# y-scope/pinot

Measured on AMD Instinct MI355X. Metric: scanned rows/sec + achieved HBM GB/s, filtered SUM on 1B-row segment, higher is better.
Workload: dtype int64

## Files before the change

### pinot_amd/csrc/pg_engine.hip

```cpp
#include <hip/hip_runtime.h>

#include <algorithm>
#include <chrono>
#include <array>
#include <atomic>
#include <condition_variable>
#include <functional>
#include <memory>
#include <cmath>
#include <cstdarg>
#include <cstdio>
#include <cstdlib>
#include <cstring>
#include <limits>
#include <mutex>
#include <string>
#include <thread>
#include <vector>

#include "../../include/pinot_gpu.h"
#include "pg_device.h"
#include "pg_filter_stats.h"
#include "pg_filter_fsm.h"
#include "pg_fsm_kernels.h"
#include "pg_kernels.h"
#include "pg_launch.h"
#include "pg_rank_image.h"
#include "pg_raw_set_table.h"

namespace {

using namespace pg;

thread_local std::string g_error;

pg_status fail(pg_status st, const char* fmt, ...) {
  char buf[1024];
  va_list ap;
  va_start(ap, fmt);
  vsnprintf(buf, sizeof(buf), fmt, ap);
  va_end(ap);
  g_error = buf;
  return st;
}

#define HIP_TRY(expr)                                                                                  \
  do {                                                                                                 \
    hipError_t _e = (expr);                                                                            \
    if (_e != hipSuccess)                                                                              \
      return fail(_e == hipErrorOutOfMemory ? PG_ERR_OUT_OF_MEMORY : PG_ERR_DEVICE, "%s failed: %s (%s:%d)", #expr, \
                  hipGetErrorString(_e), __FILE__, __LINE__);                                          \
  } while (0)

struct Engine {
  bool initialized = false;
  std::atomic<uint64_t> epoch{0};
  int device = 0;
  int blocks_per_cu = 0;
  bool raw64_coalesced = true;
  int wide_plane = -1;
  bool partition_stats_cache = true;
  bool partition_packed = true;
  bool plane_async = true;
  bool staged_h2d = true;
  long long exact_stats_docs = 64ll << 20;
  int flags = 0;
  bool use_dma = true;
  int value_plane = -1;
  int tile_steps = 0;
  bool double_buffer = false;
  bool direct_result = true;
  int fold_finalize = -1;
  int fold_one_counter = 1;
  bool poll_result = true;
  bool distinct_lds = true;
  bool set_lds = true;
  bool lane_skip = true;
  bool batch_blocks_per_cu_forced = false;
  int batch_blocks_per_cu = 4;
  bool scan_raw = true;
  bool scan_raw_set = true;
  int scan_simple_valid = 1;
  bool scan_simple = true;
  bool scan_sparse = true;
  bool lean_batch = true;
  bool partition_two_level = true;
  bool fsm_perm = true;
  int index_and_waves = 0;
  bool batch_index = true;
  bool index_gather = true;
  bool fsm_fused = true;
  bool fsm_stats = true;
  bool fsm_episodes = true;
  bool plan_cache = true;
  bool group_publish = true;
  bool batch_more = true;
  bool group_one_launch = true;
  bool batch_group = true;
  bool batch_hist = true;
  bool batch_launch = true;
  bool leap2 = true;
  int sparse_lanes = 32;
  bool plane_gcd = true;
  bool scan_private = true;
  bool group_private = true;
  int group_log_replicas = 3;
  bool group_pack = true;
  bool scan_typed_private = true;
  bool scan_narrow_single = true;
  bool scan_narrow = true;
  bool group_partition = true;
  long long partition_min_docs = 1ll << 22;
  unsigned long long group_table_bytes = 64ull << 30;
  int hist = -1;
  int hist_blocks = 0;
  bool hist_guard = false;
  int hist_bits = 0;
  int group_waves = 0;
  int physical_devices = 1;
  int logical_devices = 1;
  std::mutex mu;
};
Engine g_engine;
inline int phys_device(int logical) { return (g_engine.logical_devices > g_engine.physical_devices && g_engine.physical_devices > 0) ? logical % g_engine.physical_devices : logical; }
inline bool device_id_ok(int id) {
  if (id < 0) return false;
  if (g_engine.initialized) return id < g_engine.logical_devices;
  int n = 0;
  return hipGetDeviceCount(&n) == hipSuccess && id < n;
}

inline uint32_t be32(const uint8_t* p) { return ((uint32_t)p[0] << 24) | ((uint32_t)p[1] << 16) | ((uint32_t)p[2] << 8) | (uint32_t)p[3]; }
inline uint32_t le16(const uint8_t* p) { return (uint32_t)p[0] | ((uint32_t)p[1] << 8); }
inline uint32_t le32(const uint8_t* p) { return (uint32_t)p[0] | ((uint32_t)p[1] << 8) | ((uint32_t)p[2] << 16) | ((uint32_t)p[3] << 24); }

struct ColumnDev {
  std::string name;
  int stored_type = 0, encoding = 0, bits = 0, cardinality = 0;
  uint8_t* d_fwd_alloc = nullptr;
  uint8_t* d_fwd = nullptr;
  size_t fwd_alloc_bytes = 0;
  int32_t* d_dict = nullptr;
  std::vector<int32_t> h_dict;
  int vkind = kValI32;
  int64_t value_base = 0;
  std::vector<double> h_dict_f64;
  std::vector<int64_t> h_dict_i64;
  unsigned long long* d_dict64 = nullptr;
  uint8_t* d_inv = nullptr;
  uint64_t inv_size = 0;
  DevContainer* d_dir = nullptr;
  std::vector<DevContainer> h_dir;
  std::vector<int64_t> posting_first;
  std::vector<int64_t> posting_docs;
  unsigned long long* d_null_bitmap = nullptr;
  int nullkey_column = -1;
  int keyimage_column = -1;
  int64_t raw_min = 0, raw_max = -1;
  int key_image_of = -1;
  int64_t key_base = 0;
  int key_image_state = 0;
  bool rank_image = false;
  std::vector<unsigned long long> h_rank_keys;
  unsigned long long* d_rank_dict = nullptr;
  bool borrows_dictionary = false;
// ... 1542 lines not shown
  return v;
}

bool dict_ends_in_nan(const ColumnDev& col) {
  return col.encoding == PG_FWD_FIXED_BIT_DICT && (col.vkind == kValF64 || col.vkind == kValF32) && !col.h_dict_f64.empty() && std::isnan(col.h_dict_f64.back());
}
double group_key64_to_double(const ColumnDev& col, long long key, bool is_min) {
  if (col.vkind != kValI64 && key == (is_min ? 0x7FFFFFFFFFFFFFFFll : (long long)0x8000000000000000ull))
    return is_min ? std::numeric_limits<double>::infinity() : -std::numeric_limits<double>::infinity();
  return key64_to_double(col, key);
}

inline void cpu_relax() {
#if defined(__x86_64__) || defined(__i386__)
  __builtin_ia32_pause();
#elif defined(__aarch64__)
  asm volatile("yield" ::: "memory");
#else
  std::this_thread::yield();
#endif
}

template <typename Done>
pg_status wait_polled(hipStream_t stream, long long docs, Done&& done) {
  long long spins = 0;
  std::chrono::steady_clock::time_point until;
  while (!done()) {
    cpu_relax();
    if ((++spins & 0x3FF) != 0) continue;
    const auto now = std::chrono::steady_clock::now();
    if (spins == 0x400) { until = now + std::chrono::nanoseconds(300'000 + docs / 1000); continue; }
    if (now >= until || hipStreamQuery(stream) != hipErrorNotReady) { HIP_TRY(hipStreamSynchronize(stream)); break; }
  }
  __atomic_thread_fence(__ATOMIC_ACQUIRE);
  return PG_OK;
}

}

extern "C" {

const char* pg_last_error(void) { return g_error.c_str(); }
const char* pg_version(void) { return "pinot_amd 0.1 (gfx950)"; }

pg_status pg_init(const pg_config* config) {
  std::lock_guard<std::mutex> lk(g_engine.mu);
  if (config && config->abi_version != PG_ABI_VERSION) return fail(PG_ERR_INVALID_ARGUMENT, "ABI version mismatch: got %d, built %d", config->abi_version, PG_ABI_VERSION);
  int count = 0;
  hipError_t e = hipGetDeviceCount(&count);
  if (e != hipSuccess || count == 0) return fail(PG_ERR_DEVICE, "no HIP device available: %s", hipGetErrorString(e));
  g_engine.physical_devices = count;
  const char* ald = getenv("PINOT_GPU_ALIAS_DEVICES");
  g_engine.logical_devices = (ald && atoi(ald) > count) ? std::min(atoi(ald), 64) : count;
  int dev = config ? config->device_id : 0;
  if (dev < 0 || dev >= g_engine.logical_devices) return fail(PG_ERR_INVALID_ARGUMENT, "device %d out of range (have %d)", dev, g_engine.logical_devices);
  g_engine.device = dev;
  g_engine.blocks_per_cu = config ? config->blocks_per_cu : 0;
  g_engine.flags = config ? config->flags : 0;
  const char* nodma = getenv("PINOT_GPU_NO_DMA");
  g_engine.use_dma = !(nodma && nodma[0] == '1');
  const char* vp = getenv("PINOT_GPU_VALUE_PLANE");
  g_engine.value_plane = vp ? atoi(vp) : -1;
  const char* db = getenv("PINOT_GPU_DOUBLE_BUFFER");
  g_engine.double_buffer = db && db[0] == '1';
  const char* drv = getenv("PINOT_GPU_DIRECT_RESULT");
  g_engine.direct_result = !(drv && drv[0] == '0');
  const char* ffz = getenv("PINOT_GPU_FOLD_FINALIZE");
  g_engine.fold_finalize = ffz ? (ffz[0] == '0' ? 0 : 1) : -1;
  const char* foc = getenv("PINOT_GPU_FOLD_ONE_COUNTER");
  g_engine.fold_one_counter = foc ? (foc[0] == '0' ? 0 : 1) : 1;
  const char* prs = getenv("PINOT_GPU_POLL_RESULT");
  g_engine.poll_result = !(prs && prs[0] == '0');
  const char* lsk = getenv("PINOT_GPU_LANE_SKIP");
  g_engine.lane_skip = !(lsk && lsk[0] == '0');
  const char* bbc = getenv("PINOT_GPU_BATCH_BLOCKS_PER_CU");
  g_engine.batch_blocks_per_cu_forced = bbc != nullptr;
  g_engine.batch_blocks_per_cu = (bbc && atoi(bbc) > 0) ? atoi(bbc) : 4;
  const char* ssp = getenv("PINOT_GPU_SCAN_SPARSE");
  g_engine.scan_sparse = !(ssp && ssp[0] == '0');
  const char* ssm = getenv("PINOT_GPU_SCAN_SIMPLE");
  g_engine.scan_simple = !(ssm && ssm[0] == '0');
  const char* ssv = getenv("PINOT_GPU_SCAN_SIMPLE_VALID");
  g_engine.scan_simple_valid = ssv ? (ssv[0] == '0' ? 0 : (ssv[0] == '2' ? 2 : 1)) : 1;
  const char* srw = getenv("PINOT_GPU_SCAN_RAW");
  g_engine.scan_raw = !(srw && srw[0] == '0');
  const char* srs = getenv("PINOT_GPU_SCAN_RAW_SET");
  g_engine.scan_raw_set = !(srs && srs[0] == '0');
  const char* bla = getenv("PINOT_GPU_BATCH_LAUNCH");
  g_engine.batch_launch = !(bla && bla[0] == '0');
  auto env_on = [](const char* name) { const char* v = getenv(name); return !(v && v[0] == '0'); };
  g_engine.lean_batch = env_on("PINOT_GPU_LEAN_BATCH");
  g_engine.set_lds = env_on("PINOT_GPU_SET_LDS");
  g_engine.distinct_lds = env_on("PINOT_GPU_DISTINCT_LDS");
  g_engine.partition_two_level = env_on("PINOT_GPU_PARTITION_TWO_LEVEL");
  g_engine.fsm_perm = env_on("PINOT_GPU_FSM_PERM");
  g_engine.fsm_stats = env_on("PINOT_GPU_FSM_STATS");
  g_engine.fsm_fused = env_on("PINOT_GPU_FSM_FUSED");
  g_engine.fsm_episodes = env_on("PINOT_GPU_FSM_EPISODES");
  g_engine.index_gather = env_on("PINOT_GPU_INDEX_GATHER");
  g_engine.batch_index = env_on("PINOT_GPU_BATCH_INDEX");
  { const char* iaw = getenv("PINOT_GPU_INDEX_AND_WAVES"); g_engine.index_and_waves = iaw ? std::max(-64, std::min(32, atoi(iaw))) : 0; }
  g_engine.group_one_launch = env_on("PINOT_GPU_GROUP_ONE_LAUNCH");
  g_engine.plan_cache = env_on("PINOT_GPU_PLAN_CACHE");
  g_engine.group_publish = env_on("PINOT_GPU_GROUP_PUBLISH");
  const char* bmo = getenv("PINOT_GPU_BATCH_MORE");
  g_engine.batch_more = !(bmo && bmo[0] == '0');
  const char* bgr = getenv("PINOT_GPU_BATCH_GROUP");
  g_engine.batch_group = !(bgr && bgr[0] == '0');
  const char* bhi = getenv("PINOT_GPU_BATCH_HIST");
  g_engine.batch_hist = !(bhi && bhi[0] == '0');
  const char* lp2 = getenv("PINOT_GPU_LEAP2");
  g_engine.leap2 = !(lp2 && lp2[0] == '0');
  const char* spl = getenv("PINOT_GPU_SPARSE_LANES");
  g_engine.sparse_lanes = spl ? std::max(0, std::min(64, atoi(spl))) : 32;
  const char* pgv = getenv("PINOT_GPU_PLANE_GCD");
  g_engine.plane_gcd = !(pgv && pgv[0] == '0');
  const char* spv = getenv("PINOT_GPU_SCAN_PRIVATE");
  g_engine.scan_private = !(spv && spv[0] == '0');
  const char* gpv = getenv("PINOT_GPU_GROUP_PRIVATE");
  g_engine.group_private = !(gpv && gpv[0] == '0');
  const char* grv = getenv("PINOT_GPU_GROUP_REPLICAS");
  g_engine.group_log_replicas = grv ? std::max(0, std::min(4, atoi(grv))) : 3;
  const char* stp = getenv("PINOT_GPU_SCAN_TYPED_PRIVATE");
  g_engine.scan_typed_private = !(stp && stp[0] == '0');
  const char* gpt = getenv("PINOT_GPU_GROUP_PARTITION");
  g_engine.group_partition = !(gpt && gpt[0] == '0');
  g_engine.partition_min_docs = (gpt && gpt[0] == 'f') ? 0 : (1ll << 22);
  const char* sns = getenv("PINOT_GPU_SCAN_NARROW_SINGLE");
  g_engine.scan_narrow_single = !(sns && sns[0] == '0');
  const char* snw = getenv("PINOT_GPU_SCAN_NARROW");
  g_engine.scan_narrow = !(snw && snw[0] == '0');
  const char* gtb = getenv("PINOT_GPU_GROUP_TABLE_BYTES");
  g_engine.group_table_bytes = (gtb && atoll(gtb) > 0) ? (unsigned long long)atoll(gtb) : (64ull << 30);
  const char* gpk = getenv("PINOT_GPU_GROUP_PACK");
  g_engine.group_pack = !(gpk && gpk[0] == '0');
  const char* gw = getenv("PINOT_GPU_GROUP_WAVES");
  g_engine.group_waves = (gw && atoi(gw) > 0) ? atoi(gw) : 0;
  const char* hs = getenv("PINOT_GPU_HIST");
  g_engine.hist = hs ? atoi(hs) : -1;
  const char* hbl = getenv("PINOT_GPU_HIST_BLOCKS");
  g_engine.hist_blocks = (hbl && atoi(hbl) > 0) ? atoi(hbl) : 0;
  const char* hg = getenv("PINOT_GPU_HIST_GUARD");
  g_engine.hist_guard = hg && hg[0] == '1';
  const char* hb = getenv("PINOT_GPU_HIST_BITS");
  g_engine.hist_bits = (hb && (atoi(hb) == 8 || atoi(hb) == 16)) ? atoi(hb) : 0;
  const char* ts = getenv("PINOT_GPU_TILE_STEPS");
  g_engine.tile_steps = (ts && (atoi(ts) == 16 || atoi(ts) == 32)) ? atoi(ts) : 0;
  g_engine.raw64_coalesced = true; g_engine.wide_plane = -1; g_engine.partition_stats_cache = true; g_engine.partition_packed = true;
  g_engine.plane_async = true; g_engine.staged_h2d = true; g_engine.exact_stats_docs = 64ll << 20;
  const char* r64 = getenv("PINOT_GPU_RAW64_COALESCED");
  if (r64) g_engine.raw64_coalesced = atoi(r64) != 0;
  const char* wpl = getenv("PINOT_GPU_WIDE_PLANE");
  if (wpl) g_engine.wide_plane = atoi(wpl);
  const char* psc = getenv("PINOT_GPU_PARTITION_STATS_CACHE");
  if (psc) g_engine.partition_stats_cache = atoi(psc) != 0;
  const char* ppk = getenv("PINOT_GPU_PARTITION_PACKED");
  if (ppk) g_engine.partition_packed = atoi(ppk) != 0;
  const char* pas = getenv("PINOT_GPU_PLANE_ASYNC");
  if (pas) g_engine.plane_async = atoi(pas) != 0;
  const char* sh2d = getenv("PINOT_GPU_STAGED_H2D");
  if (sh2d) g_engine.staged_h2d = atoi(sh2d) != 0;
  {
    uint64_t budget = config ? config->plane_budget_bytes : 0;
    const char* pb = getenv("PINOT_GPU_PLANE_BUDGET_BYTES");
    if (pb) budget = strtoull(pb, nullptr, 10);
    if (budget == 0) {
// ... 681 lines not shown
  std::shared_ptr<IndexAndParams> and_params;
  uint32_t and_windows = 0;
  size_t hist_lds = 0;
  int hist_cw = 0, hist_col = -1;
  std::string key;
  uint64_t engine_epoch = 0, plane_epoch = 0;
  std::shared_ptr<const OwnedQuery> query;
};
struct Deferred {
  std::shared_ptr<const LoweredItem> item;
  std::unique_ptr<PlaneHold> planes;
  bool cacheable = false;
  bool single = false;
};

static bool query_key(const pg_query* q, std::string* key) {
  key->clear();
  if (q->num_filter_nodes < 0 || q->num_predicates < 0 || q->num_aggregations < 0 || q->num_group_by < 0) return false;
  if ((q->num_filter_nodes > 0 && !q->filter) || (q->num_predicates > 0 && !q->predicates) || (q->num_aggregations > 0 && !q->aggregations) ||
      (q->num_group_by > 0 && !q->group_by_columns)) return false;
  const int32_t head[6] = {q->num_filter_nodes, q->num_predicates, q->num_aggregations, q->num_group_by, q->num_groups_limit, q->flags};
  key->append(reinterpret_cast<const char*>(head), sizeof(head));
  key->append(reinterpret_cast<const char*>(q->filter), sizeof(pg_filter_node) * (size_t)q->num_filter_nodes);
  for (int i = 0; i < q->num_predicates; ++i) {
    const pg_predicate& pr = q->predicates[i];
    if (pr.num_set_words < 0 || (pr.num_set_words > 0 && !pr.set_words)) { key->clear(); return false; }
    const int64_t fields[8] = {pr.kind, pr.column, pr.eval, pr.exclusive, pr.lo, pr.hi, pr.num_set_words, pr.reserved};
    key->append(reinterpret_cast<const char*>(fields), sizeof(fields));
    key->append(reinterpret_cast<const char*>(pr.set_words), sizeof(uint32_t) * (size_t)pr.num_set_words);
  }
  key->append(reinterpret_cast<const char*>(q->aggregations), sizeof(pg_aggregation) * (size_t)q->num_aggregations);
  key->append(reinterpret_cast<const char*>(q->group_by_columns), sizeof(int32_t) * (size_t)q->num_group_by);
  return true;
}

static std::shared_ptr<const OwnedQuery> own_query(const pg_query* q) {
  auto o = std::make_shared<OwnedQuery>();
  o->q = *q;
  if (q->num_filter_nodes > 0) o->filter.assign(q->filter, q->filter + q->num_filter_nodes);
  if (q->num_predicates > 0) o->predicates.assign(q->predicates, q->predicates + q->num_predicates);
  o->set_words.resize(o->predicates.size());
  for (size_t i = 0; i < o->predicates.size(); ++i) {
    pg_predicate& pr = o->predicates[i];
    if (pr.num_set_words > 0) { o->set_words[i].assign(pr.set_words, pr.set_words + pr.num_set_words); pr.set_words = o->set_words[i].data(); }
    else pr.set_words = nullptr;
  }
  if (q->num_aggregations > 0) o->aggregations.assign(q->aggregations, q->aggregations + q->num_aggregations);
  o->q.filter = o->filter.empty() ? nullptr : o->filter.data();
  o->q.predicates = o->predicates.empty() ? nullptr : o->predicates.data();
  o->q.aggregations = o->aggregations.empty() ? nullptr : o->aggregations.data();
  if (q->num_group_by > 0) o->group_by.assign(q->group_by_columns, q->group_by_columns + q->num_group_by);
  o->q.group_by_columns = o->group_by.empty() ? nullptr : o->group_by.data();
  return o;
}

static pg_status prepare_fsm_side(pg_segment* seg, ExecCtx* ctx, const pg::fstats::Fsm& fsm, FsmSide* side);
static pg_status device_fsm_filter_stats(pg_segment* seg, ExecCtx* ctx, const pg_query* q, const FsmSide& side, pg_result* out);
struct ExecTrace {
  std::chrono::steady_clock::time_point t[6];
  bool seen[6];
};
static thread_local ExecTrace t_exec_trace;
static bool exec_trace_on() { static const bool on = getenv("PINOT_GPU_EXEC_TRACE") != nullptr; return on; }
static inline void exec_mark(int i) {
  if (!exec_trace_on()) return;
  t_exec_trace.t[i] = std::chrono::steady_clock::now();
  t_exec_trace.seen[i] = true;
}

static pg_status execute_impl(pg_segment* seg, const pg_query* q, pg_result* out, unsigned long long* d_out_bitmap_request,
                              uint64_t* host_bitmap, int64_t host_bitmap_words, int64_t* out_cardinality, bool allow_metadata_plan = true,
                              Deferred* defer = nullptr, FsmSide* side = nullptr);

enum class ScanKernel { Hist, Narrow, NarrowSingle, Sparse, Simple, SimpleSet, SimpleValid, Raw, RawSet, PrivateFsm, Private, PrivateTyped, Distinct, GroupDistinct, Agg };
static const struct { int id; bool writes_leaves; } kScanKernels[] = {
  {PG_KERNEL_SCAN_HIST, true}, {PG_KERNEL_SCAN_NARROW, true}, {PG_KERNEL_SCAN_NARROW, false}, {PG_KERNEL_SCAN_SPARSE, false}, {PG_KERNEL_SCAN_SIMPLE, false},
  {PG_KERNEL_SCAN_SIMPLE, false}, {PG_KERNEL_SCAN_SIMPLE_VALID, false}, {PG_KERNEL_SCAN_RAW, false}, {PG_KERNEL_SCAN_RAW_SET, false}, {PG_KERNEL_SCAN_PRIVATE, false}, {PG_KERNEL_SCAN_PRIVATE, true},
  {PG_KERNEL_SCAN_PRIVATE_TYPED, true}, {PG_KERNEL_SCAN_DISTINCT, true}, {PG_KERNEL_GROUP_DISTINCT, true}, {PG_KERNEL_SCAN_AGG, false}};
static_assert(sizeof(kScanKernels) / sizeof(kScanKernels[0]) == (size_t)ScanKernel::Agg + 1, "one row per ScanKernel");
struct ScanChoice {
  ScanKernel kernel = ScanKernel::Agg, general = ScanKernel::Agg;
  int hist_slot = -1, hist_cw = 0;
  bool hist_guarded = false;
};
static ScanChoice choose_scan_kernel(const pg_segment* seg, const Lowered& lw, int hist_col, bool typed, bool want_bitmap, bool want_result) {
  const PlanParams& pl = lw.plan; const ScanParams& sp = lw.sp;
  const bool profile = (g_engine.flags & PG_CFG_PROFILE_WAVES) != 0;
  ScanChoice k;
  auto pick = [&k](ScanKernel kernel) { k.kernel = kernel; return k; };
  if (sp.num_nodes == 1 && sp.nodes[0].op == PG_FILTER_LEAF && sp.nodes[0].kind == kLeafRawSet) { k.general = ScanKernel::Private; return pick(ScanKernel::RawSet); }
  if (!lw.distinct_slots.empty()) { k.general = ScanKernel::Private; return pick(lw.distinct_key_slots.empty() ? ScanKernel::Distinct : ScanKernel::GroupDistinct); }
  bool private_leaves = true;
  for (int l = 0; l < pl.num_leaves; ++l) private_leaves &= pl.leaves[l].kind <= kLeafBitmap || pl.leaves[l].kind == kLeafDocRange;
  bool lane_private = g_engine.scan_private && !typed && !profile && private_leaves;
  for (int i = 0; i < pl.num_agg_cols && hist_col >= 0; ++i) if (lw.col_of_slot[(size_t)pl.agg_cols[i].col] == hist_col * 2) k.hist_slot = i;
  for (int i = 0; i < pl.num_agg_cols && lane_private; ++i) {
    const DevColumn& c = pl.cols[pl.agg_cols[i].col];
    lane_private = !c.is_raw && c.vkind == kValI32 && c.bits <= 31 && (!pl.agg_cols[i].need_sum || c.is_plane || i == k.hist_slot);
  }
  const bool hist = lane_private && k.hist_slot == 0 && pl.num_agg_cols == 1;
  if (k.hist_slot >= 0 && !hist) lane_private = false;
  bool lane_typed = g_engine.scan_private && g_engine.scan_typed_private && !lane_private && pl.num_agg_cols > 0 && !profile && private_leaves;
  for (int i = 0; i < pl.num_agg_cols && lane_typed; ++i) {
    const DevColumn& c = pl.cols[pl.agg_cols[i].col];
    lane_typed = c.is_raw || (c.vkind != kValI32 && c.bits <= 31);
  }
  k.general = k.kernel = lane_private ? ScanKernel::Private : (lane_typed ? ScanKernel::PrivateTyped : ScanKernel::Agg);
  if (hist) {
    k.hist_cw = hist_counter_bits(seg->cols[(size_t)hist_col]);
    k.hist_guarded = std::max(__atomic_load_n(&seg->cols[(size_t)hist_col].hist_tier, __ATOMIC_RELAXED), g_engine.hist_guard ? 1 : 0) >= 1 && k.hist_cw < 32;
    return pick(ScanKernel::Hist);
  }
  if (k.general == ScanKernel::Agg) return k;
  if (g_engine.scan_narrow && lane_private && pl.num_agg_cols == 0 && lw.tile_list == nullptr && sp.num_nodes > 0 && !(want_result && lw.stats_leap2_flagged)) {
    bool narrow = true; int depth = 0, max_depth = 0;
    for (int n = 0; n < sp.num_nodes && narrow; ++n) {
      const DevNode& dn = sp.nodes[n];
      if (dn.op == PG_FILTER_LEAF) {
        narrow = dn.kind == kLeafMatchAll || dn.kind == kLeafMatchNone || ((dn.kind == kLeafDictRange || (dn.kind == kLeafDictSet && g_engine.set_lds)) && dn.bits >= 1 && dn.bits <= kNarrowMaxBits);
        depth++;
      } else if (dn.op != PG_FILTER_NOT) depth -= dn.num_children - 1;
      max_depth = std::max(max_depth, depth);
    }
    if (narrow && max_depth <= kNarrowStack)
      return pick(g_engine.scan_narrow_single && sp.num_nodes == 1 && sp.nodes[0].kind == kLeafDictRange ? ScanKernel::NarrowSingle : ScanKernel::Narrow);
  }
  if (g_engine.scan_sparse && lane_private && !want_bitmap && pl.num_agg_cols > 0 && lw.tile_list != nullptr && sp.num_nodes == 1 && sp.nodes[0].kind == kLeafBitmap &&
      sp.nodes[0].exclusive == 0) return pick(ScanKernel::Sparse);
  if (g_engine.scan_simple_valid != 0 && g_engine.scan_simple && lane_private && !want_bitmap && lw.tile_list == nullptr && lw.side == nullptr && lw.valid_leaf >= 0 &&
      pl.num_agg_cols <= 1 && !lw.stats_leap2_flagged && (sp.num_nodes == 1 || sp.num_nodes == 3)) {
    const DevNode& v = sp.nodes[0];
    const DevNode* range = sp.num_nodes == 3 ? &sp.nodes[1] : nullptr;
    const DevAggCol* vac = pl.num_agg_cols == 1 ? &sp.agg_cols[0] : nullptr;
    bool valid = v.op == PG_FILTER_LEAF && v.kind == kLeafBitmap && v.exclusive == 0 && v.set_words == reinterpret_cast<const uint32_t*>(pl.leaves[lw.valid_leaf].bitmap) &&
                 (range != nullptr || vac != nullptr);
    if (valid && range != nullptr)
      valid = sp.nodes[2].op == PG_FILTER_AND && sp.nodes[2].num_children == 2 && range->op == PG_FILTER_LEAF && range->kind == kLeafDictRange && range->bits >= 1 && range->bits <= kSimpleMaxBits &&
              (range->flags & kNodeLeapfrog2) == 0;
    if (valid && vac != nullptr)
      valid = vac->bits >= 1 && vac->bits <= kSimpleMaxBits && !vac->is_raw &&
              !(range != nullptr && range->fwd == vac->fwd && range->bits == vac->bits && vac->need_sum != 0 && vac->need_minmax == 0 && range->exclusive == 0);
    if (valid) return pick(ScanKernel::SimpleValid);
  }
  if (want_bitmap || lw.tile_list != nullptr || sp.num_nodes > 1 || pl.num_agg_cols > 1 || (want_result && (lw.stats_leap2_flagged || lw.stats_chain_flagged))) return k;
  const DevNode* leaf = sp.num_nodes == 1 ? &sp.nodes[0] : nullptr;
  const bool plain_leaf = leaf == nullptr || (leaf->op == PG_FILTER_LEAF && (leaf->flags & (kNodeCountEntries | kNodeLeapfrog2)) == 0);
  const DevAggCol* ac = pl.num_agg_cols == 1 ? &sp.agg_cols[0] : nullptr;
  const bool set = leaf != nullptr && leaf->op == PG_FILTER_LEAF && leaf->kind == kLeafDictSet && g_engine.set_lds && leaf->bits <= 16;
  bool simple = g_engine.scan_simple && lane_private && plain_leaf &&
                (leaf == nullptr || ((leaf->kind == kLeafDictRange || set) && leaf->bits >= 1 && leaf->bits <= kSimpleMaxBits));
  if (simple && ac != nullptr)
    simple = ac->bits >= 1 && ac->bits <= kSimpleMaxBits && !ac->is_raw && !(leaf != nullptr && leaf->fwd == ac->fwd && leaf->bits == ac->bits && ac->need_sum != 0 && ac->need_minmax == 0 && leaf->exclusive == 0);
  if (simple) return pick(set ? ScanKernel::SimpleSet : ScanKernel::Simple);
  if (g_engine.scan_raw && lw.side == nullptr && sp.num_nodes + pl.num_agg_cols >= 1 && plain_leaf && (leaf == nullptr || (leaf->kind == kLeafRawRange && leaf->fwd != nullptr)) &&
      (ac == nullptr || (ac->is_raw != 0 && ac->vkind == kValI32 && ac->is_plane == 0 && ac->bits == 32))) return pick(ScanKernel::Raw);
  return k;
}
struct ScanGrid { int blocks = 1, threads = kBlockThreads; size_t lds = 0, hist_set_off = 0; bool wide = false, distinct_lds = false; };
static void lean_grid(const pg_segment* seg, int wave_cap, ScanGrid* g) {
  const long long tiles2k = doc_tiles(seg);
  static const bool wide_ok = getenv("PINOT_GPU_WIDE_BLOCKS") && getenv("PINOT_GPU_WIDE_BLOCKS")[0] == '1';
  g->wide = wide_ok && wave_cap >= 2 * (kWideBlockThreads / 64) && tiles2k > 64 && tiles2k <= (long long)seg->num_cus * wave_cap && g_engine.blocks_per_cu <= 0;
  const int wpb = (g->wide ? kWideBlockThreads : kBlockThreads) / 64;
  int bpc = std::max(1, wave_cap / wpb);
  static const int small_bpc = getenv("PINOT_GPU_SMALL_BLOCKS_PER_CU") ? atoi(getenv("PINOT_GPU_SMALL_BLOCKS_PER_CU")) : 2;
  if (!g->wide && small_bpc > 0 && tiles2k <= 2ll * seg->num_cus * wave_cap) bpc = std::min(bpc, small_bpc);
  g->blocks = grid_blocks(seg, tiles2k, wpb, bpc);
}
static ScanGrid scan_grid(const pg_segment* seg, const ScanChoice& k, const Lowered& lw, const Geometry& geo, int num_agg_cols, int hist_col) {
  const ScanParams& sp = lw.sp;
  ScanGrid g;
  const long long tiles = doc_tiles(seg);
  const int wpb = kBlockThreads / 64, hist_waves = kHistBlockThreads / 64;
  switch (k.kernel) {
    case ScanKernel::Hist: {
      const int per_word = 32 / k.hist_cw;
      g.lds = (((size_t)(seg->cols[(size_t)hist_col].cardinality + per_word - 1) / per_word * 4) + 15) & ~(size_t)15;
      g.lds = std::max(g.lds, sizeof(BlockPartial) * (kHistBlockThreads / 64) + 16);
      if (g_engine.set_lds && g.lds + (size_t)kSetLdsWords * 4 <= 150 * 1024)
        for (int nd = 0; nd < sp.num_nodes; ++nd) if (sp.nodes[nd].op == PG_FILTER_LEAF && sp.nodes[nd].kind == kLeafDictSet) g.hist_set_off = g.lds;
      if (g.hist_set_off != 0) g.lds += (size_t)kSetLdsWords * 4;
      g.threads = kHistBlockThreads;
      g.blocks = grid_blocks(seg, tiles, hist_waves, std::max(1, std::min(waves_scan_hist(k.hist_cw, k.hist_guarded) / hist_waves, (int)((160 * 1024 - 2048) / (g.lds + 256)))));
      if (g_engine.hist_blocks > 0) g.blocks = std::min(g.blocks, g_engine.hist_blocks);
      break;
    }
    case ScanKernel::Distinct: case ScanKernel::GroupDistinct: {
      bool has_set = false;
      if (g_engine.set_lds) for (int nd = 0; nd < sp.num_nodes; ++nd) has_set |= sp.nodes[nd].op == PG_FILTER_LEAF && sp.nodes[nd].kind == kLeafDictSet;
      size_t bit_bytes = 0;
      for (int slot : lw.distinct_slots) bit_bytes += (size_t)((lw.plan.cols[slot].cardinality + 31) / 32) * 4;
      bit_bytes = (bit_bytes + 15) & ~(size_t)15;
      const size_t records = sizeof(BlockPartial) * (kHistBlockThreads / 64) + 16;
      size_t lds_tier = bit_bytes + (has_set ? (size_t)kSetLdsWords * 4 : 0);
      if (lds_tier > kLdsBudget && bit_bytes <= kLdsBudget) { has_set = false; lds_tier = bit_bytes; }
      g.distinct_lds = k.kernel == ScanKernel::Distinct && g_engine.distinct_lds && std::max(lds_tier, records) <= kLdsBudget;
      if (g.distinct_lds) {
        g.hist_set_off = has_set ? bit_bytes : 0;
        g.lds = std::max(lds_tier, records);
        g.threads = kHistBlockThreads;
        g.blocks = grid_blocks(seg, tiles, hist_waves, std::max(1, std::min(waves_scan_distinct(true) / hist_waves, (int)((160 * 1024 - 2048) / (g.lds + 256)))));
      } else {
        g.hist_set_off = has_set ? 16 : 0;
        g.lds = std::max((size_t)(has_set ? 16 + kSetLdsWords * 4 : 0), sizeof(BlockPartial) * (size_t)wpb + 16);
        g.blocks = grid_blocks(seg, tiles, wpb, std::max(1, (k.kernel == ScanKernel::Distinct ? waves_scan_distinct(false) : waves_group_distinct()) / wpb));
      }
      break;
    }
    case ScanKernel::Narrow: g.blocks = grid_blocks(seg, (tiles + kNarrowTiles - 1) / kNarrowTiles, wpb, std::max(1, waves_scan_narrow(false) / wpb)); break;
    case ScanKernel::NarrowSingle: g.blocks = grid_blocks(seg, (tiles + kNarrowSingleTiles - 1) / kNarrowSingleTiles, wpb, std::max(1, waves_scan_narrow(true) / wpb)); break;
    case ScanKernel::Sparse: g.blocks = grid_blocks(seg, tiles, wpb * kSparseTiles, std::max(1, waves_scan_sparse(num_agg_cols <= 1) / wpb)); break;
    case ScanKernel::Simple: case ScanKernel::SimpleSet: lean_grid(seg, waves_scan_simple(), &g); break;
    case ScanKernel::SimpleValid: lean_grid(seg, waves_scan_simple_valid(), &g); break;
    case ScanKernel::Raw: lean_grid(seg, waves_scan_raw(), &g); break;
    case ScanKernel::RawSet: {
      g.lds = (size_t)sp.nodes[0].set_bytes;
      int bpc = std::max(1, std::min(waves_scan_raw_set(sp.nodes[0].lo_hi) / wpb, (int)(kLdsBudget / (g.lds + 1024))));
      if (tiles <= 2ll * seg->num_cus * bpc * wpb) bpc = std::min(bpc, 2);
      g.blocks = grid_blocks(seg, tiles, wpb, bpc);
      break;
    }
    case ScanKernel::Private: g.blocks = grid_blocks(seg, tiles, wpb, std::max(1, waves_scan_private(num_agg_cols) / wpb)); break;
    case ScanKernel::PrivateTyped: g.blocks = grid_blocks(seg, tiles, wpb, std::max(1, waves_scan_private_typed(num_agg_cols) / wpb)); break;
    default: g.blocks = geo.blocks; g.threads = geo.threads; g.lds = geo.lds; break;
  }
  return g;
}
static bool scan_batch_kind(const ScanChoice& k, int num_agg_cols, BatchKind* kind) {
  const bool lean = g_engine.lean_batch;
  switch (k.kernel) {
    case ScanKernel::Hist: *kind = k.hist_cw == 8 ? BatchKind::Hist8 : (k.hist_cw == 16 ? BatchKind::Hist16 : BatchKind::Hist32); return !k.hist_guarded && g_engine.batch_hist;
    case ScanKernel::Narrow: case ScanKernel::NarrowSingle: *kind = k.kernel == ScanKernel::Narrow ? BatchKind::Narrow : BatchKind::NarrowSingle; return g_engine.batch_more;
    case ScanKernel::Simple: case ScanKernel::SimpleSet: *kind = !lean ? BatchKind::Private : (k.kernel == ScanKernel::Simple ? BatchKind::Simple : BatchKind::SimpleSet); return true;
    case ScanKernel::Raw: *kind = !lean && k.general == ScanKernel::Private ? BatchKind::Private : BatchKind::Raw; return true;
    case ScanKernel::RawSet: return false;
    case ScanKernel::SimpleValid: return false;
    case ScanKernel::PrivateFsm: case ScanKernel::Private: *kind = BatchKind::Private; return true;
    case ScanKernel::PrivateTyped: *kind = num_agg_cols <= 1 ? BatchKind::Typed1 : (num_agg_cols == 2 ? BatchKind::Typed2 : BatchKind::TypedMax); return g_engine.batch_more;
    default: return false;
  }
}
static void launch_scan_kernel(const ScanChoice& k, const ScanGrid& g, int num_agg_cols, bool typed, hipStream_t stream, const ScanParams& sp) {
  const bool one = num_agg_cols <= 1;
  const int lean_threads = g.wide ? kWideBlockThreads : kBlockThreads;
  switch (k.kernel) {
    case ScanKernel::Hist: launch_scan_hist(k.hist_cw, k.hist_guarded, g.blocks, g.lds, stream, sp); break;
    case ScanKernel::Narrow: case ScanKernel::NarrowSingle: launch_scan_narrow(k.kernel == ScanKernel::NarrowSingle, g.blocks, stream, sp); break;
    case ScanKernel::Sparse: launch_scan_sparse(one, g.blocks, stream, sp); break;
    case ScanKernel::Simple: case ScanKernel::SimpleSet: launch_scan_simple(g.blocks, lean_threads, stream, sp, k.kernel == ScanKernel::SimpleSet); break;
    case ScanKernel::SimpleValid: launch_scan_simple_valid(g.blocks, lean_threads, stream, sp, g_engine.scan_simple_valid == 2); break;
    case ScanKernel::Raw: launch_scan_raw(g.blocks, lean_threads, stream, sp); break;
    case ScanKernel::RawSet: launch_scan_raw_set(sp.nodes[0].lo_hi, g.blocks, g.lds, stream, sp); break;
    case ScanKernel::PrivateFsm: launch_scan_private_fsm(num_agg_cols, g.blocks, stream, sp); break;
    case ScanKernel::Private: launch_scan_private(num_agg_cols, g.blocks, stream, sp); break;
    case ScanKernel::PrivateTyped: launch_scan_private_typed(num_agg_cols, g.blocks, stream, sp); break;
    case ScanKernel::Agg: launch_scan_agg(g_engine.use_dma, one, typed, g.blocks, g.threads, g.lds, stream, sp); break;
    case ScanKernel::Distinct: case ScanKernel::GroupDistinct: break;
  }
}
struct QueryRun {
  pg_segment* seg; const pg_query* q; pg_result* out; ExecCtx* ctx; Deferred* defer;
  int na, ng, hist_col = -1;
  bool want_bitmap, timed, stats_is_final = false;
  Lowered lw;
  PlaneHold planes;
  std::vector<int> projected;
  QueryRun(pg_segment* s, const pg_query* q_, pg_result* o, ExecCtx* c, Deferred* d, int na_, int ng_, bool want_bitmap_, bool timed_)
      : seg(s), q(q_), out(o), ctx(c), defer(d), na(na_), ng(ng_), want_bitmap(want_bitmap_), timed(timed_), planes(s, {}) {}
  void add_projected(int c) { if (std::find(projected.begin(), projected.end(), c) == projected.end()) projected.push_back(c); }
};
static pg_status defer_item(QueryRun& r, std::shared_ptr<LoweredItem> item) {
  item->plane_columns = r.planes.columns;
  item->doc_sets = r.lw.doc_sets;
  r.defer->item = std::move(item);
  r.defer->cacheable = !r.lw.plane_pending;
  r.defer->planes.reset(new PlaneHold(std::move(r.planes)));
  return kDeferred;
}
static std::shared_ptr<LoweredItem> index_and_item(const Lowered& lw) {
  auto item = std::make_shared<LoweredItem>();
  memset(&item->sp, 0, sizeof(item->sp));
  item->sp.lean_kind = (int32_t)BatchKind::IndexAnd;
  item->and_params = std::make_shared<IndexAndParams>(lw.and_params);
  item->and_windows = lw.finalize_windows;
  item->blocks = (int)std::min<long long>(((long long)lw.finalize_windows + index_and_batch_block_waves() - 1) / index_and_batch_block_waves(), (long long)lw.and_num_cus * index_and_batch_blocks_per_cu());
  return item;
}
static void empty_agg_value(pg_agg_value* v, int64_t count) { v->count = count; v->min = std::numeric_limits<double>::infinity(); v->max = -std::numeric_limits<double>::infinity(); }
static void nothing_scanned(pg_result* o, int64_t docs, int total_docs) {
  o->stats.num_docs_scanned = docs; o->stats.num_entries_scanned_in_filter = 0; o->filter_entries_exact = 1; o->stats.num_entries_scanned_post_filter = 0; o->stats.num_total_docs = total_docs;
}
static void start_group_result(pg_result* out, int na, int ng, int num_present, int kernel, int upper_bound, int key_kind) {
  out->num_aggregations = na; out->dominant_kernel = kernel; out->num_groups = num_present; out->group_id_upper_bound = upper_bound;
  out->group_ids = (int32_t*)malloc(sizeof(int32_t) * (size_t)std::max(num_present, 1));
  out->group_aggregations = (pg_agg_value*)calloc((size_t)std::max(num_present, 1) * (size_t)std::max(na, 1), sizeof(pg_agg_value));
  out->group_key_dict_ids = (int32_t*)malloc(sizeof(int32_t) * (size_t)std::max(num_present, 1) * (size_t)ng);
  out->group_key_kind = key_kind;
}
static pg_status time_index_and(const ExecCtx* ctx, pg_result* out) {
  float ms_all = 0.f;
  HIP_TRY(hipEventElapsedTime(&ms_all, ctx->ev[0], ctx->ev[3]));
  out->device_ms = ms_all; out->dominant_kernel_ms = ms_all;
  return PG_OK;
}
static bool answer_from_metadata(const pg_segment* seg, const pg_query* q, int na, pg_result* out, int64_t* out_cardinality) {
  bool match_all = q->num_filter_nodes == 0;
  if (q->num_filter_nodes == 1 && q->filter && q->predicates && q->filter[0].op == PG_FILTER_LEAF && q->filter[0].predicate >= 0 &&
      q->filter[0].predicate < q->num_predicates) {
    const pg_predicate& pr = q->predicates[q->filter[0].predicate];
    match_all = (pr.kind == PG_PRED_MATCH_ALL && !pr.exclusive) || (pr.kind == PG_PRED_MATCH_NONE && pr.exclusive);
  }
  bool fit = match_all;
  for (int a = 0; a < na && fit; ++a) {
    const pg_aggregation& ag = q->aggregations[a];
    if (ag.function == PG_AGG_COUNT) continue;
    fit = (ag.function == PG_AGG_MIN || ag.function == PG_AGG_MAX) && ag.column >= 0 && ag.column < (int)seg->cols.size() &&
          seg->cols[(size_t)ag.column].encoding == PG_FWD_FIXED_BIT_DICT;
  }
  if (!fit) return false;
  memset(out, 0, sizeof(*out));
  out->num_aggregations = na;
  out->aggregations = (pg_agg_value*)calloc((size_t)na, sizeof(pg_agg_value));
  for (int a = 0; a < na; ++a) {
    const pg_aggregation& ag = q->aggregations[a];
    pg_agg_value& v = out->aggregations[a];
    empty_agg_value(&v, seg->num_docs);
    if (ag.function == PG_AGG_MIN) v.min = seg->cols[(size_t)ag.column].h_dict_f64.front();
    if (ag.function == PG_AGG_MAX) v.max = seg->cols[(size_t)ag.column].h_dict_f64.back();
  }
  nothing_scanned(out, seg->num_docs, seg->num_docs);
  if (out_cardinality) *out_cardinality = seg->num_docs;
  return true;
// ... 2767 lines not shown
```

### pinot_amd/csrc/pg_launch.h

```cpp
#ifndef PG_LAUNCH_H
#define PG_LAUNCH_H
#include <hip/hip_runtime.h>

#include <algorithm>

#include "pg_device.h"

namespace pg {

template <typename K>
int max_waves_per_cu(K kernel) {
  hipFuncAttributes attr;
  if (hipFuncGetAttributes(&attr, reinterpret_cast<const void*>(kernel)) != hipSuccess || attr.numRegs <= 0) return 16;
  const int alloc = ((attr.numRegs + 7) / 8) * 8;
  return std::max(1, std::min(6, 512 / alloc)) * 4;
}
template <typename K>
int max_waves_per_cu_lean(K kernel) {
  hipFuncAttributes attr;
  if (hipFuncGetAttributes(&attr, reinterpret_cast<const void*>(kernel)) != hipSuccess || attr.numRegs <= 0) return 16;
  const int alloc = ((attr.numRegs + 7) / 8) * 8;
  return std::max(1, std::min(8, 512 / alloc)) * 4;
}
template <typename K>
void set_dynamic_lds(K kernel, size_t bytes) {
  if (bytes > 48 * 1024) (void)hipFuncSetAttribute(reinterpret_cast<const void*>(kernel), hipFuncAttributeMaxDynamicSharedMemorySize, (int)bytes);
}

void launch_scan_agg(bool dma, bool one_slot, bool typed, int blocks, int threads, size_t lds, hipStream_t stream, const ScanParams& p);
int waves_scan_agg(bool one_slot, bool typed);
void launch_scan_private(int agg_cols, int blocks, hipStream_t stream, const ScanParams& p);
int waves_scan_private(int agg_cols);
void launch_scan_private_fsm(int agg_cols, int blocks, hipStream_t stream, const ScanParams& p);
int waves_scan_private_fsm(int agg_cols);
void launch_scan_private_batch(bool one_slot, int total_blocks, hipStream_t stream, const ScanParams* items, const uint32_t* block_first, int num_items);
void launch_scan_sparse(bool one_slot, int blocks, hipStream_t stream, const ScanParams& p);
int waves_scan_sparse(bool one_slot);
void launch_scan_simple(int blocks, int threads, hipStream_t stream, const ScanParams& p, bool set_leaf = false);
int waves_scan_simple();
void launch_scan_simple_valid(int blocks, int threads, hipStream_t stream, const ScanParams& p, bool skip_empty_tiles);
int waves_scan_simple_valid();
void launch_scan_raw(int blocks, int threads, hipStream_t stream, const ScanParams& p);
int waves_scan_raw();
void launch_scan_raw_set(int key_bytes, int blocks, size_t table_bytes, hipStream_t stream, const ScanParams& p);
int waves_scan_raw_set(int key_bytes);
void launch_raw_set_bitmap(int key_bytes, int blocks, hipStream_t stream, const RawSetBitmapParams& p);
int waves_raw_set_bitmap(int key_bytes);
void launch_scan_lean_batch(int kind, int total_blocks, hipStream_t stream, const ScanParams* items, const uint32_t* block_first, int num_items);
int waves_scan_lean_batch(int kind);
void launch_scan_narrow(bool single_leaf, int blocks, hipStream_t stream, const ScanParams& p);
int waves_scan_narrow(bool single_leaf);
void launch_scan_narrow_batch(bool single_leaf, int total_blocks, hipStream_t stream, const ScanParams* items, const uint32_t* block_first, int num_items);
int waves_scan_narrow_batch(bool single_leaf);
void launch_scan_typed_batch(int agg_slots, int total_blocks, hipStream_t stream, const ScanParams* items, const uint32_t* block_first, int num_items);
int waves_scan_typed_batch(int agg_slots);
void launch_index_and_kernel(int blocks, hipStream_t stream, const IndexAndParams& ap, uint32_t num_windows);
int waves_index_and();
int index_and_batch_blocks_per_cu();
int index_and_batch_block_waves();
void launch_index_and_batch(int total_blocks, hipStream_t stream, const IndexAndParams* items, const uint32_t* block_first, int num_items);
void launch_scan_group(bool dma, bool lds_table, int blocks, int threads, size_t lds, hipStream_t stream, const GroupParams& gp);
int waves_scan_group();
void launch_group_private(bool lds_table, int blocks, int threads, size_t lds, hipStream_t stream, const GroupParams& gp);
int waves_group_private();
void launch_group_lds_batch(int total_blocks, int threads, size_t lds, hipStream_t stream, const GroupParams* items, const uint32_t* block_first, int num_items);
int waves_group_lds_batch();

void launch_scan_hist(int counter_bits, bool guarded, int blocks, size_t lds, hipStream_t stream, const ScanParams& p);
int waves_scan_hist(int counter_bits, bool guarded);
void launch_scan_hist_batch(int counter_bits, int total_blocks, size_t lds, hipStream_t stream, const ScanParams* items, const uint32_t* block_first, int num_items);
int waves_scan_hist_batch(int counter_bits);

void launch_scan_distinct(bool lds_tier, int blocks, size_t lds, hipStream_t stream, const DistinctParams& dp);
int waves_scan_distinct(bool lds_tier);
void launch_group_distinct(int blocks, size_t lds, hipStream_t stream, const DistinctParams& dp);
int waves_group_distinct();

void launch_scan_private_typed(int agg_cols, int blocks, hipStream_t stream, const ScanParams& p);
int waves_scan_private_typed(int agg_cols);
void launch_group_partition_histogram(int blocks, hipStream_t stream, const PartitionParams& pp);
void launch_group_partition_scatter(int blocks, hipStream_t stream, const PartitionParams& pp);
void launch_group_partition_aggregate(int work_items, size_t lds, hipStream_t stream, const PartitionParams& pp);
void launch_group_repartition(int num_chunks, hipStream_t stream, const RepartitionParams& rp);
void launch_group_typed_direct(int blocks, hipStream_t stream, const GroupParams& gp);
int waves_group_partition_scatter();
int blocks_per_cu_group_partition_scatter_packed(int num_partitions);

}
#endif
```

Before: 1677 billion.

## Add software-pipelined simple scan kernel prefetching next filter tile

Adds a new simple-scan kernel variant that loads each lane's packed filter words with a few 16-byte vector loads and prefetches the next tile's filter words while the current tile's value words are loaded and aggregated. The engine picks it by default for single dict-range leaf plus one aggregate column when the filter's estimated selectivity is at least a threshold. The aim is to hide global-memory latency with register double-buffering and wide loads. The cost is more registers per lane, which may lower occupancy, and a large set of template instantiations.

```diff
diff --git a/pinot_amd/csrc/pg_engine.hip b/pinot_amd/csrc/pg_engine.hip
--- a/pinot_amd/csrc/pg_engine.hip
+++ b/pinot_amd/csrc/pg_engine.hip
@@ -81,6 +81,7 @@
   bool scan_raw = true;
   bool scan_raw_set = true;
   int scan_simple_valid = 1;
+  int scan_simple_pipe = 1;
   bool scan_simple = true;
   bool scan_sparse = true;
   bool lean_batch = true;
@@ -1789,6 +1790,8 @@
   g_engine.scan_simple = !(ssm && ssm[0] == '0');
   const char* ssv = getenv("PINOT_GPU_SCAN_SIMPLE_VALID");
   g_engine.scan_simple_valid = ssv ? (ssv[0] == '0' ? 0 : (ssv[0] == '2' ? 2 : 1)) : 1;
+  const char* spp = getenv("PINOT_GPU_SCAN_SIMPLE_PIPE");
+  g_engine.scan_simple_pipe = spp ? (spp[0] == '0' ? 0 : (spp[0] == '2' ? 2 : 1)) : 1;
   const char* srw = getenv("PINOT_GPU_SCAN_RAW");
   g_engine.scan_raw = !(srw && srw[0] == '0');
   const char* srs = getenv("PINOT_GPU_SCAN_RAW_SET");
@@ -2636,7 +2639,9 @@
   ScanKernel kernel = ScanKernel::Agg, general = ScanKernel::Agg;
   int hist_slot = -1, hist_cw = 0;
   bool hist_guarded = false;
+  bool pipe = false;
 };
+constexpr int kPipeMinSelectivityPct = 5;
 static ScanChoice choose_scan_kernel(const pg_segment* seg, const Lowered& lw, int hist_col, bool typed, bool want_bitmap, bool want_result) {
   const PlanParams& pl = lw.plan; const ScanParams& sp = lw.sp;
   const bool profile = (g_engine.flags & PG_CFG_PROFILE_WAVES) != 0;
@@ -2705,6 +2710,12 @@
                 (leaf == nullptr || ((leaf->kind == kLeafDictRange || set) && leaf->bits >= 1 && leaf->bits <= kSimpleMaxBits));
   if (simple && ac != nullptr)
     simple = ac->bits >= 1 && ac->bits <= kSimpleMaxBits && !ac->is_raw && !(leaf != nullptr && leaf->fwd == ac->fwd && leaf->bits == ac->bits && ac->need_sum != 0 && ac->need_minmax == 0 && leaf->exclusive == 0);
+  if (simple && !set && leaf != nullptr && ac != nullptr && g_engine.scan_simple_pipe != 0 && scan_simple_pipe_shape(leaf->bits, ac->bits)) {
+    const DevColumn& fc = pl.cols[pl.leaves[pl.nodes[0].leaf].col];
+    const unsigned long long values = fc.is_plane ? 1ull << leaf->bits : (unsigned long long)std::max(fc.cardinality, 1);
+    const unsigned long long inside = std::min<unsigned long long>(leaf->span, values), taken = leaf->exclusive ? values - inside : inside;
+    k.pipe = g_engine.scan_simple_pipe == 2 || taken * 100ull >= (unsigned long long)kPipeMinSelectivityPct * values;
+  }
   if (simple) return pick(set ? ScanKernel::SimpleSet : ScanKernel::Simple);
   if (g_engine.scan_raw && lw.side == nullptr && sp.num_nodes + pl.num_agg_cols >= 1 && plain_leaf && (leaf == nullptr || (leaf->kind == kLeafRawRange && leaf->fwd != nullptr)) &&
       (ac == nullptr || (ac->is_raw != 0 && ac->vkind == kValI32 && ac->is_plane == 0 && ac->bits == 32))) return pick(ScanKernel::Raw);
@@ -2764,7 +2775,7 @@
     case ScanKernel::Narrow: g.blocks = grid_blocks(seg, (tiles + kNarrowTiles - 1) / kNarrowTiles, wpb, std::max(1, waves_scan_narrow(false) / wpb)); break;
     case ScanKernel::NarrowSingle: g.blocks = grid_blocks(seg, (tiles + kNarrowSingleTiles - 1) / kNarrowSingleTiles, wpb, std::max(1, waves_scan_narrow(true) / wpb)); break;
     case ScanKernel::Sparse: g.blocks = grid_blocks(seg, tiles, wpb * kSparseTiles, std::max(1, waves_scan_sparse(num_agg_cols <= 1) / wpb)); break;
-    case ScanKernel::Simple: case ScanKernel::SimpleSet: lean_grid(seg, waves_scan_simple(), &g); break;
+    case ScanKernel::Simple: case ScanKernel::SimpleSet: lean_grid(seg, k.pipe ? waves_scan_simple_pipe() : waves_scan_simple(), &g); break;
     case ScanKernel::SimpleValid: lean_grid(seg, waves_scan_simple_valid(), &g); break;
     case ScanKernel::Raw: lean_grid(seg, waves_scan_raw(), &g); break;
     case ScanKernel::RawSet: {
@@ -2801,7 +2812,10 @@
     case ScanKernel::Hist: launch_scan_hist(k.hist_cw, k.hist_guarded, g.blocks, g.lds, stream, sp); break;
     case ScanKernel::Narrow: case ScanKernel::NarrowSingle: launch_scan_narrow(k.kernel == ScanKernel::NarrowSingle, g.blocks, stream, sp); break;
     case ScanKernel::Sparse: launch_scan_sparse(one, g.blocks, stream, sp); break;
-    case ScanKernel::Simple: case ScanKernel::SimpleSet: launch_scan_simple(g.blocks, lean_threads, stream, sp, k.kernel == ScanKernel::SimpleSet); break;
+    case ScanKernel::Simple: case ScanKernel::SimpleSet:
+      if (k.pipe) launch_scan_simple_pipe(g.blocks, lean_threads, stream, sp);
+      else launch_scan_simple(g.blocks, lean_threads, stream, sp, k.kernel == ScanKernel::SimpleSet);
+      break;
     case ScanKernel::SimpleValid: launch_scan_simple_valid(g.blocks, lean_threads, stream, sp, g_engine.scan_simple_valid == 2); break;
     case ScanKernel::Raw: launch_scan_raw(g.blocks, lean_threads, stream, sp); break;
     case ScanKernel::RawSet: launch_scan_raw_set(sp.nodes[0].lo_hi, g.blocks, g.lds, stream, sp); break;
diff --git a/pinot_amd/csrc/pg_launch.h b/pinot_amd/csrc/pg_launch.h
--- a/pinot_amd/csrc/pg_launch.h
+++ b/pinot_amd/csrc/pg_launch.h
@@ -38,6 +38,9 @@
 int waves_scan_sparse(bool one_slot);
 void launch_scan_simple(int blocks, int threads, hipStream_t stream, const ScanParams& p, bool set_leaf = false);
 int waves_scan_simple();
+bool scan_simple_pipe_shape(int filter_bits, int value_bits);
+void launch_scan_simple_pipe(int blocks, int threads, hipStream_t stream, const ScanParams& p);
+int waves_scan_simple_pipe();
 void launch_scan_simple_valid(int blocks, int threads, hipStream_t stream, const ScanParams& p, bool skip_empty_tiles);
 int waves_scan_simple_valid();
 void launch_scan_raw(int blocks, int threads, hipStream_t stream, const ScanParams& p);
diff --git a/pinot_amd/csrc/pg_scan_simple_pipe.h b/pinot_amd/csrc/pg_scan_simple_pipe.h
--- /dev/null
+++ b/pinot_amd/csrc/pg_scan_simple_pipe.h
@@ -0,0 +1,132 @@
+#pragma once
+#include "pg_scan_simple.h"
+
+namespace pg {
+
+static_assert((kSimpleMaxBits + 3) / 4 == 5, "scan_simple_pipe_kernel is instantiated for one to five 16-byte loads per column");
+
+typedef uint32_t Dword4 __attribute__((ext_vector_type(4), aligned(4)));
+
+template <int N4>
+__device__ __forceinline__ int pipe_tail_back(int lane, int bits) {
+  const int over = lane * bits + 4 * N4 - 64 * bits;
+  return over > 0 ? over : 0;
+}
+
+template <int N4>
+__device__ __forceinline__ void pipe_load_chunk(GlobalWords tile_words, uint32_t at, uint32_t tail, uint32_t (&r)[4 * N4]) {
+#pragma unroll
+  for (int i = 0; i < N4; ++i) {
+    const Dword4 q = *(const __attribute__((address_space(1))) Dword4*)(i == N4 - 1 ? tile_words + tail : tile_words + at + 4 * i);
+    r[4 * i + 0] = q.x; r[4 * i + 1] = q.y; r[4 * i + 2] = q.z; r[4 * i + 3] = q.w;
+  }
+}
+
+template <int N4, int K>
+__device__ __forceinline__ void pipe_align_tail(uint32_t (&r)[4 * N4], int back) {
+  constexpr int t = 4 * (N4 - 1);
+  if (K >= 1) {
+    const bool one = (back & 1) != 0;
+    r[t + 0] = one ? r[t + 1] : r[t + 0]; r[t + 1] = one ? r[t + 2] : r[t + 1]; r[t + 2] = one ? r[t + 3] : r[t + 2];
+  }
+  if (K >= 2) {
+    const bool two = (back & 2) != 0;
+    r[t + 0] = two ? r[t + 2] : r[t + 0]; r[t + 1] = two ? r[t + 3] : r[t + 1];
+  }
+}
+
+template <int N4, bool kLoZero>
+__device__ __forceinline__ uint32_t pipe_range_dispatch(int b, uint32_t (&r)[4 * N4], int back, uint32_t lo, uint32_t span) {
+  uint32_t m = 0;
+  const uint32_t* words = r;
+  switch (b) {
+#define PG_CASE(K) case 4 * N4 - K: pipe_align_tail<N4, K>(r, back); range16_private<4 * N4 - K, 0, kLoZero>(words, lo, span, m); range16_private<4 * N4 - K, 1, kLoZero>(words, lo, span, m); break;
+    PG_CASE(3) PG_CASE(2) PG_CASE(1) PG_CASE(0)
+#undef PG_CASE
+    default: break;
+  }
+  return __builtin_bitreverse32(m);
+}
+
+template <int N4>
+__device__ __forceinline__ void pipe_agg_dispatch(int b, uint32_t (&r)[4 * N4], int back, uint32_t m, bool need_sum, bool need_minmax,
+                                                  uint32_t& psum, unsigned long long& wsum, uint32_t& umin, uint32_t& umax) {
+  const uint32_t* words = r;
+  switch (b) {
+#define PG_CASE(K) case 4 * N4 - K: pipe_align_tail<N4, K>(r, back); agg16_private<4 * N4 - K, 0>(words, m, need_sum, need_minmax, psum, wsum, umin, umax); \
+                                    agg16_private<4 * N4 - K, 1>(words, m, need_sum, need_minmax, psum, wsum, umin, umax); break;
+    PG_CASE(3) PG_CASE(2) PG_CASE(1) PG_CASE(0)
+#undef PG_CASE
+    default: break;
+  }
+}
+
+template <int NF4, int NV4, typename P>
+__device__ __forceinline__ void pipe_tile(const P& p, long long tile, int lane, uint32_t (&fw)[4 * NF4], uint32_t (&vw)[4 * NV4], int backs,
+                                          unsigned long long& count, unsigned long long& sum, uint32_t& umin, uint32_t& umax) {
+  const auto& L = p.nodes[0];
+  const auto& ac = p.agg_cols[0];
+  uint32_t m = L.lo == 0 ? pipe_range_dispatch<NF4, true>(L.bits, fw, backs, 0u, L.span) : pipe_range_dispatch<NF4, false>(L.bits, fw, backs, (uint32_t)L.lo, L.span);
+  if (L.exclusive) m = ~m;
+  const long long rem = (long long)p.num_docs - (tile * 2048 + lane * 32);
+  m &= rem >= 32 ? 0xFFFFFFFFu : (rem <= 0 ? 0u : ((1u << (int)rem) - 1u));
+  count += (unsigned)__builtin_popcount(m);
+  uint32_t psum = 0, tmin = 0xFFFFFFFFu, tmax = 0u;
+  unsigned long long wsum = 0;
+  pipe_agg_dispatch<NV4>(ac.bits, vw, backs >> 2, m, ac.need_sum != 0, ac.need_minmax != 0, psum, wsum, tmin, tmax);
+  sum += wsum + psum;
+  umin = tmin < umin ? tmin : umin;
+  umax = tmax > umax ? tmax : umax;
+}
+
+template <int NF4, int NV4, typename P>
+__device__ __forceinline__ void scan_simple_pipe_body(const P& p, uint32_t block_index, uint32_t num_blocks, BlockPartial* red, uint32_t* fold_flag_ptr) {
+  const int lane = threadIdx.x & 63;
+  const int wave_in_block = __builtin_amdgcn_readfirstlane((int)(threadIdx.x >> 6));
+  const int waves_per_block = blockDim.x >> 6;
+  const long long total_waves = (long long)num_blocks * waves_per_block;
+  const long long num_tiles = ((long long)p.num_docs + 2047) / 2048;
+  const auto& L = p.nodes[0];
+  const auto& ac = p.agg_cols[0];
+  const GlobalWords f_words = global_words(L.fwd), v_words = global_words(ac.fwd);
+  const long long f_tile_words = 64ll * L.bits, v_tile_words = 64ll * ac.bits;
+  const int fback = pipe_tail_back<NF4>(lane, L.bits), vback = pipe_tail_back<NV4>(lane, ac.bits);
+  const int backs = fback | vback << 2;
+  const uint32_t f_at = (uint32_t)(lane * L.bits), f_tail = f_at + 4u * (NF4 - 1) - (uint32_t)fback;
+  const uint32_t v_at = (uint32_t)(lane * ac.bits), v_tail = v_at + 4u * (NV4 - 1) - (uint32_t)vback;
+
+  unsigned long long count = 0, sum = 0;
+  uint32_t umin = 0xFFFFFFFFu, umax = 0u;
+  long long tile = (long long)block_index * waves_per_block + wave_in_block;
+  if (tile < num_tiles) {
+    uint32_t fw[4 * NF4];
+    pipe_load_chunk<NF4>(f_words + tile * f_tile_words, f_at, f_tail, fw);
+    for (long long next = tile + total_waves; next < num_tiles; next += total_waves) {
+      uint32_t vw[4 * NV4], fn[4 * NF4];
+      pipe_load_chunk<NV4>(v_words + tile * v_tile_words, v_at, v_tail, vw);
+      pipe_load_chunk<NF4>(f_words + next * f_tile_words, f_at, f_tail, fn);
+      __builtin_amdgcn_sched_barrier(0);
+      pipe_tile<NF4, NV4>(p, tile, lane, fw, vw, backs, count, sum, umin, umax);
+#pragma unroll
+      for (int i = 0; i < 4 * NF4; ++i) fw[i] = fn[i];
+      tile = next;
+    }
+    uint32_t vw[4 * NV4];
+    pipe_load_chunk<NV4>(v_words + tile * v_tile_words, v_at, v_tail, vw);
+    __builtin_amdgcn_sched_barrier(0);
+    pipe_tile<NF4, NV4>(p, tile, lane, fw, vw, backs, count, sum, umin, umax);
+  }
+
+  BlockPartial mine;
+  partial_identity(mine);
+  mine.count = (unsigned long long)wave_sum_i64((long long)count);
+  mine.sum[0] = wave_sum_i64((long long)sum);
+  mine.kmin[0] = wave_min_i32(umin == 0xFFFFFFFFu ? 0x7FFFFFFF : (int32_t)umin);
+  mine.kmax[0] = wave_max_i32(count == 0ull ? (int32_t)0x80000000 : (int32_t)umax);
+  if (lane == 0) red[wave_in_block] = mine;
+  __syncthreads();
+  publish_block_partial(p, red, waves_per_block, fold_flag_ptr, block_index, num_blocks);
+}
+
+
+}
diff --git a/pinot_amd/csrc/pg_unit_scan_simple_pipe.hip b/pinot_amd/csrc/pg_unit_scan_simple_pipe.hip
--- /dev/null
+++ b/pinot_amd/csrc/pg_unit_scan_simple_pipe.hip
@@ -0,0 +1,41 @@
+#include "pg_scan_simple_pipe.h"
+#include "pg_launch.h"
+
+namespace pg {
+
+template <int NF4, int NV4>
+__global__ __launch_bounds__(kWideBlockThreads, PG_SIMPLE_WAVES) void scan_simple_pipe_kernel(const ScanParams p) {
+  __shared__ BlockPartial red[kWideBlockThreads / 64];
+  __shared__ uint32_t fold_flag;
+  scan_simple_pipe_body<NF4, NV4>(p, blockIdx.x, gridDim.x, red, &fold_flag);
+}
+
+typedef void (*PipeKernel)(const ScanParams);
+#define K(F, V) scan_simple_pipe_kernel<F, V>
+static const PipeKernel kPipeKernels[5][5] = {{K(1, 1), K(1, 2), K(1, 3), K(1, 4), K(1, 5)},
+                                              {K(2, 1), K(2, 2), K(2, 3), K(2, 4), K(2, 5)},
+                                              {K(3, 1), K(3, 2), K(3, 3), K(3, 4), K(3, 5)},
+                                              {K(4, 1), K(4, 2), K(4, 3), K(4, 4), nullptr},
+                                              {K(5, 1), K(5, 2), nullptr, nullptr, nullptr}};
+#undef K
+
+bool scan_simple_pipe_shape(int filter_bits, int value_bits) {
+  if (filter_bits < 1 || filter_bits > kSimpleMaxBits || value_bits < 1 || value_bits > kSimpleMaxBits) return false;
+  return kPipeKernels[(filter_bits + 3) / 4 - 1][(value_bits + 3) / 4 - 1] != nullptr;
+}
+
+void launch_scan_simple_pipe(int blocks, int threads, hipStream_t stream, const ScanParams& p) {
+  const int nf4 = (p.nodes[0].bits + 3) / 4, nv4 = (p.agg_cols[0].bits + 3) / 4;
+  kPipeKernels[nf4 - 1][nv4 - 1]<<<dim3((unsigned)blocks), dim3((unsigned)threads), 0, stream>>>(p);
+}
+
+int waves_scan_simple_pipe() {
+  static const int cap = [] {
+    int least = max_waves_per_cu_lean(kPipeKernels[0][0]);
+    for (int f = 0; f < 5; ++f) for (int v = 0; v < 5; ++v) if (kPipeKernels[f][v] != nullptr) least = std::min(least, max_waves_per_cu_lean(kPipeKernels[f][v]));
+    return least;
+  }();
+  return cap;
+}
+
+}
```

Measured after the change: 1750 billion, median of 6. 1.04x the previous value.
